# spectralcode/OCTproZ

Measured on AMD Instinct MI355X. Metric: A-scans/s, higher is better.
Workload: dtype f32

## Files before the change

octproz_amd/csrc/kernels.h:

```cpp
#pragma once
#ifndef __HIPCC_RTC__
#include <hip/hip_runtime.h>
#endif
#include <stdint.h>

#include "fft_regs.h"

namespace oct {

enum { IN_U8 = 0, IN_U16 = 1, IN_U32 = 2, IN_F32 = 3, IN_P12U = 4, IN_P12S = 5, IN_I16 = 6 };
enum { RS_NONE = 0, RS_LINEAR = 1, RS_CUBIC = 2, RS_LANCZOS = 3 };

struct FusedArgs {
	const void* raw;
	float* out;
	f2* spectrum;
	const float4* lut;
	const f2* twiddle;
	const f2* meanLine;
	unsigned numLines;
	unsigned linesInBuffer;
	unsigned ascansPerBscan;
	int bitshift;
	int rollingW;
// ... 350 lines not shown
		for (int m = 0; m < NB; m++) {
			const int b = lane + 64 * m;
			const int j0 = (b / NS) * (NS * R) + (b & (NS - 1));
			float* wb = plane + j0 + K * (j0 >> 5);
#pragma unroll
			for (int u = 0; u < R; u++) wb[u * NS + K * ((u * NS) >> 5)] = c ? v[m + u * NB].y : v[m + u * NB].x;
		}
		wave_sync_lds();
#pragma unroll
		for (int q = 0; q < P; q++) (c ? ny : nx)[q] = rb[(64 + 2 * K) * q];
		wave_sync_lds();
	}
#pragma unroll
	for (int q = 0; q < P; q++) v[q] = f2{nx[q], ny[q]};
}

template <int LOG2N> struct Plan;
template <> struct Plan<8>  { static constexpr int R0 = 4,  R1 = 4,  R2 = 4,  R3 = 4; static constexpr bool PERM = false; };
template <> struct Plan<9>  { static constexpr int R0 = 8,  R1 = 8,  R2 = 8,  R3 = 1; static constexpr bool PERM = false; };
template <> struct Plan<10> { static constexpr int R0 = 16, R1 = 16, R2 = 4,  R3 = 1; static constexpr bool PERM = true; };
template <> struct Plan<11> { static constexpr int R0 = 32, R1 = 16, R2 = 4,  R3 = 1; static constexpr bool PERM = false; };
template <> struct Plan<12> { static constexpr int R0 = 64, R1 = 16, R2 = 4,  R3 = 1; static constexpr bool PERM = false; };

template <int LOG2N> constexpr int twiddle_count() {
	typedef Plan<LOG2N> PL;
	int n = 0, ns = PL::R0;
	n += (PL::R1 - 1) * ns; ns *= PL::R1;
	n += (PL::R2 - 1) * ns; ns *= PL::R2;
	if (PL::R3 > 1) n += (PL::R3 - 1) * ns;
	return n;
}
template <int LOG2N> struct LastRadix { static constexpr int value = Plan<LOG2N>::R3 == 1 ? Plan<LOG2N>::R2 : Plan<LOG2N>::R3; };

OCT_DEV void perm_swap32(float& a, float& b) {
	const auto r = __builtin_amdgcn_permlane32_swap(__builtin_bit_cast(unsigned, a), __builtin_bit_cast(unsigned, b), false, false);
	const unsigned r0 = r[0], r1 = r[1];
	a = __builtin_bit_cast(float, r0);
	b = __builtin_bit_cast(float, r1);
}
OCT_DEV void perm_swap16(float& a, float& b) {
	const auto r = __builtin_amdgcn_permlane16_swap(__builtin_bit_cast(unsigned, a), __builtin_bit_cast(unsigned, b), false, false);
	const unsigned r0 = r[0], r1 = r[1];
	a = __builtin_bit_cast(float, r0);
	b = __builtin_bit_cast(float, r1);
}
OCT_DEV void perm_exchange16x4(f2 (&v)[16]) {
#pragma unroll
	for (int m = 0; m < 4; m++) {
		float x[4], y[4];
#pragma unroll
		for (int c = 0; c < 4; c++) { x[c] = v[4 * m + c].x; y[c] = v[4 * m + c].y; }
		perm_swap32(x[0], x[2]); perm_swap32(x[1], x[3]); perm_swap32(y[0], y[2]); perm_swap32(y[1], y[3]);
		perm_swap16(x[0], x[1]); perm_swap16(x[2], x[3]); perm_swap16(y[0], y[1]); perm_swap16(y[2], y[3]);
#pragma unroll
		for (int c = 0; c < 4; c++) v[4 * m + c] = f2{x[c], y[c]};
	}
	f2 w[16];
#pragma unroll
	for (int m = 0; m < 4; m++)
#pragma unroll
		for (int a = 0; a < 4; a++) w[m + 4 * a] = v[4 * m + a];
#pragma unroll
	for (int i = 0; i < 16; i++) v[i] = w[i];
}
template <int P> OCT_DEV void perm_exchange(f2 (&v)[P]) {
	if constexpr (P == 16) perm_exchange16x4(v);
}
OCT_DEV void perm_exchange32x2(f2 (&v)[32]) {
	f2 w[32];
#pragma unroll
	for (int m = 0; m < 2; m++)
#pragma unroll
		for (int mp = 0; mp < 8; mp++) {
			float ax = v[m + 4 * mp].x, ay = v[m + 4 * mp].y, bx = v[m + 4 * mp + 2].x, by = v[m + 4 * mp + 2].y;
			perm_swap32(ax, bx);
			perm_swap32(ay, by);
			w[mp + 8 * (2 * m)] = f2{ax, ay};
			w[mp + 8 * (2 * m + 1)] = f2{bx, by};
		}
#pragma unroll
	for (int i = 0; i < 32; i++) v[i] = w[i];
}

template <int LOG2N> OCT_DEV int fft_bin(int lane, int m, int u) {
	constexpr int N = 1 << LOG2N, RL = LastRadix<LOG2N>::value;
	return lane + 64 * m + u * (N / RL);
}
template <int LOG2N, bool PRUNE, bool REGTW = false, bool REGTW3 = false, int PRIO2 = -1>
OCT_DEV void fft_wave(f2 (&v)[(1 << LOG2N) / 64], f2* xbuf, const f2* tw, int lane, const f32x4* twr = nullptr) {
	constexpr int N = 1 << LOG2N;
	typedef Plan<LOG2N> PL;
	constexpr int R0 = PL::R0, R1 = PL::R1, R2 = PL::R2, R3 = PL::R3;
	static_assert(R0 * R1 * R2 * R3 == N, "plan");
	constexpr int T1 = 0, T2 = T1 + (R1 - 1) * R0, T3 = T2 + (R2 - 1) * R0 * R1;
	constexpr int P = N / 64;
	if constexpr (Cfg<LOG2N>::PLANAR) {
		static_assert(R1 == 16 && R2 == 4 && R3 == 1 && P == R0, "planar plans: P x 16 x 4 with the whole first pass in the lane");
		float* plane = reinterpret_cast<float*>(xbuf);
		fft_pass<N, R0, 1, false, false, false>(v, xbuf, tw, lane);
		exchange_planar<N, R0>(v, plane, lane);
		fft_pass<N, R1, R0, false, false, false>(v, xbuf, tw + T1, lane);
		if constexpr (P == 32) {
			perm_exchange32x2(v);
		} else {
			f2 w[P];
#pragma unroll
			for (int m = 0; m < 4; m++)
#pragma unroll
				for (int u = 0; u < 16; u++) w[(u + 16 * m) % P] = v[(m + 4 * u) % P];
#pragma unroll
			for (int i = 0; i < P; i++) v[i] = w[i];
		}
		fft_pass<N, R2, R0 * R1, false, false, PRUNE>(v, xbuf, tw + T2, lane);
		return;
	}
	fft_pass<N, R0, 1, false, true, false>(v, xbuf, tw, lane);
	if constexpr (PL::PERM) {
		static_assert(!PL::PERM || (R3 == 1 && R2 == 4 && R1 == 16 && P == 16), "permlane exchange: 16-point lanes, radix 16 then 4");
		fft_pass<N, R1, R0, true, false, false, 2, REGTW, false, PRIO2>(v, xbuf, tw, lane, twr);
		perm_exchange<P>(v);
		fft_pass<N, R2, R0 * R1, false, false, PRUNE, 3, REGTW, REGTW3>(v, xbuf, tw + 8 * 16 * 2, lane, twr);
	} else if constexpr (R3 == 1) {
		fft_pass<N, R1, R0, true, true, false>(v, xbuf, tw + T1, lane);
		fft_pass<N, R2, R0 * R1, true, false, PRUNE>(v, xbuf, tw + T2, lane);
	} else {
		fft_pass<N, R1, R0, true, true, false>(v, xbuf, tw + T1, lane);
		fft_pass<N, R2, R0 * R1, true, true, false>(v, xbuf, tw + T2, lane);
		fft_pass<N, R3, R0 * R1 * R2, true, false, PRUNE>(v, xbuf, tw + T3, lane);
	}
}

template <int LOG2N> constexpr int tw_lds_bytes() { return Plan<LOG2N>::PERM ? (8 * 16 + 6 * 64) * 16 : (twiddle_count<LOG2N>() * 8 + 15) & ~15; }
template <int LOG2N>
OCT_DEV void fill_twiddles(f2* tw, const f2* g, int tid, int threads) {
	if constexpr (Plan<LOG2N>::PERM) {
		typedef Plan<LOG2N> PL;
		constexpr int T2 = (PL::R1 - 1) * PL::R0;
		f32x4* p2 = reinterpret_cast<f32x4*>(tw);
		f32x4* p3 = p2 + 8 * 16;
		for (int i = tid; i < 8 * 16; i += threads) {
			const int c = i >> 4, k = i & 15;
			const f2 w0 = c ? g[(2 * c - 1) * 16 + k] : f2{1.0f, 0.0f}, w1 = g[(2 * c) * 16 + k];
			p2[i] = f32x4{w0.x, w0.y, w1.x, w1.y};
		}
		for (int i = tid; i < 6 * 64; i += threads) {
			const int c = i >> 6, l = i & 63, i0 = 2 * c, i1 = 2 * c + 1;
			const f2 w0 = g[T2 + (i0 % 3) * 256 + l + 64 * (i0 / 3)], w1 = g[T2 + (i1 % 3) * 256 + l + 64 * (i1 / 3)];
			p3[i] = f32x4{w0.x, w0.y, w1.x, w1.y};
		}
	} else {
		for (int i = tid; i < twiddle_count<LOG2N>(); i += threads) tw[i] = g[i];
	}
}
template <int LOG2N, int RS> constexpr int mean_lds_bytes() { return KCfg<LOG2N, RS>::MEAN_REGS ? 0 : (1 << LOG2N) * 4; }
template <int LOG2N, int RS, bool ROLL = false> constexpr int lut_lds_bytes() { return (!Cfg<LOG2N>::LDS_LUT || KCfg<LOG2N, RS>::REGTAB || KCfg<LOG2N, RS, ROLL>::REGLIN) ? 0 : (1 << LOG2N) * (KCfg<LOG2N, RS>::CW ? 24 : 12) + (KCfg<LOG2N, RS>::LZ_LDS ? (1 << LOG2N) * 64 : 0); }
template <int LOG2N, int RS, bool ROLL> constexpr int block_lds_bytes() {
	return tw_lds_bytes<LOG2N>() + mean_lds_bytes<LOG2N, RS>() + lut_lds_bytes<LOG2N, RS, ROLL>() + KCfg<LOG2N, RS, ROLL>::WAVES * wave_lds_bytes<(1 << LOG2N), ROLL>();
}

OCT_DEV unsigned flipped_row(const FusedArgs& a, unsigned line) {
	const unsigned b = line / a.ascansPerBscan, as = line - b * a.ascansPerBscan;
	return ((b & 1u) == 0u && (b + 2u) * a.ascansPerBscan <= a.linesInBuffer) ? b * a.ascansPerBscan + (a.ascansPerBscan - 1u - as) : line;
}
template <bool> OCT_DEV void ef_flush(const FusedArgs& a, float acc, unsigned first, unsigned stride, int lane, unsigned count) {
	if ((unsigned)lane < count) {
		const unsigned line = first + (unsigned)lane * stride;
		a.dispEnFace[a.dispEnFaceLast - (a.flip ? flipped_row(a, line) : line)] = acc;
	}
}

enum { MODE_ROLL = 1, MODE_SPECTRUM = 2, MODE_LOG = 4, MODE_BG = 8, MODE_DISP = 16, MODE_SINUS = 32 };
template <int MODE, int LOG2N, int RS> constexpr int sinus_lds_bytes() {
	constexpr bool ROLL = (MODE & MODE_ROLL) != 0;
	constexpr int want = KCfg<LOG2N, RS, ROLL>::WAVES * (1 << LOG2N) * 2;
	return (MODE & MODE_SINUS) != 0 && block_lds_bytes<LOG2N, RS, ROLL>() + bg_lds_bytes<MODE, (1 << LOG2N)>() + want <= 160 * 1024 ? want : 0;
}
template <int MODE, int LOG2N, int RS> constexpr bool sinus_prev_lds() { return sinus_lds_bytes<MODE, LOG2N, RS>() > 0; }
OCT_DEV float sinus_blend(float f0, float f1, float frac) {
#pragma clang fp contract(off)
	const float d = f1 - f0;
	const float t = d * frac;
	return f0 + t;
}

struct SinusWalk {
	typedef const __attribute__((address_space(4))) u32x4 ent_t;
	ent_t* ent;
	unsigned M, total, blk, A, lines, units;
	int flip;
	unsigned sBlk, sT, sTEnd, sI2, sBA, sBA0, sBB, next;
	bool sFl;
	u32x4 e0, e1, e2;
	OCT_DEV bool flipped(unsigned bb) const { return flip && (bb & 1u) == 0u && (bb + 2u) * A <= lines; }
	OCT_DEV unsigned row(unsigned ba, bool fl, uint32_t x) const { const unsigned pp = x & 0xffffu; return ba + (fl ? A - 1u - pp : pp); }
	OCT_DEV unsigned wrap(unsigned i) const { return i + 1u == M ? 0u : i + 1u; }
	OCT_DEV bool valid() const { return sBlk * blk + 1u < total; }
	OCT_DEV unsigned enter() {
		const unsigned g0 = sBlk * blk, last = total - 1u;
		sTEnd = min(blk, last - g0);
		sT = 0;
		const unsigned bb = g0 / M, i0 = g0 - bb * M, i1 = wrap(i0);
		e0 = ent[i0];
		e1 = ent[i1];
		sI2 = wrap(i1);
		sBA0 = bb * A;
		sBB = i1 == 0u ? bb + 1u : bb;
		sBA = sBB * A;
		sFl = flipped(sBB);
		return row(sBA0, flipped(bb), e0.x);
	}
	OCT_DEV unsigned begin(const FusedArgs& a, unsigned first, unsigned unitsInGrid) {
		ent = reinterpret_cast<ent_t*>(reinterpret_cast<uintptr_t>(a.sinEnt));
		M = a.sinM; total = a.sinTotal; blk = a.sinBlk; A = a.ascansPerBscan; lines = a.linesInBuffer; flip = a.flip; units = unitsInGrid;
		sBlk = first; sT = sTEnd = sI2 = sBA = sBA0 = sBB = 0; next = 0xFFFFFFFFu; sFl = false;
		e0 = e1 = e2 = u32x4{0u, 0u, 0u, 0u};
		return valid() ? enter() : 0xFFFFFFFFu;
	}
	OCT_DEV void load_ahead() { e2 = ent[sI2]; }
	OCT_DEV unsigned peek_next() { next = sT < sTEnd ? row(sBA, sFl, e1.x) : 0xFFFFFFFFu; return next; }
	OCT_DEV unsigned advance(bool* newBlock) {
		*newBlock = false;
		if (sT < sTEnd) {
			sT++;
			e0 = e1; sBA0 = sBA;
			e1 = e2;
			if (sI2 == 0u) { sBB++; sBA += A; sFl = flipped(sBB); }
			sI2 = wrap(sI2);
			return next;
		}
		sBlk += units;
		if (!valid()) return 0xFFFFFFFFu;
		*newBlock = true;
		return enter();
	}
	OCT_DEV unsigned out_row() const { return sBA0 + (e0.x >> 16); }
	OCT_DEV void pair(float* f0, float* f1, bool* st0, bool* st1, bool* raw) const {
		const uint32_t b0 = e0.y, b1 = e0.z;
		*f0 = __builtin_bit_cast(float, b0);
		*f1 = __builtin_bit_cast(float, b1);
		const unsigned r0 = out_row();
		const bool p = sT > 0u && *f0 >= 0.0f;
		*st0 = p && r0 + 1u != lines;
		*st1 = p && *f1 >= 0.0f && r0 + 2u != lines;
		*raw = sBA0 + (e0.x & 0xffffu) + 1u == lines;
	}
};

template <int LOG2N, int INTYPE, int RS, int MODE>
__global__ __launch_bounds__((KCfg<LOG2N, RS, (MODE & 1) != 0>::WAVES) * 64, (KCfg<LOG2N, RS, (MODE & 1) != 0>::MINW)) void oct_fused_kernel(const FusedArgs a) {
	constexpr int N = 1 << LOG2N, P = N / 64;
	constexpr int WAVES = KCfg<LOG2N, RS, (MODE & MODE_ROLL) != 0>::WAVES, THREADS = WAVES * 64;
	constexpr bool LDS_LUT = Cfg<LOG2N>::LDS_LUT, CW = KCfg<LOG2N, RS>::CW, MEAN_REGS = KCfg<LOG2N, RS>::MEAN_REGS, REGTAB = KCfg<LOG2N, RS>::REGTAB;
	constexpr bool REGLIN = KCfg<LOG2N, RS, (MODE & 1) != 0>::REGLIN && RS != RS_LANCZOS;
	constexpr int RL = LastRadix<LOG2N>::value, NBL = P / RL;
	constexpr bool ROLL = (MODE & MODE_ROLL) != 0, SPECTRUM = (MODE & MODE_SPECTRUM) != 0, LOGSCALE = (MODE & MODE_LOG) != 0;
	constexpr bool SINUS = (MODE & MODE_SINUS) != 0;
	static_assert(!(SINUS && (SPECTRUM || (MODE & MODE_DISP) != 0 || RS == RS_LANCZOS)), "sinusoidal correction in the store: image output of the raw-row variants, display frames by the extraction kernel");
	typedef Chunk<INTYPE, N> CH;
	constexpr int SPL = CH::SPL, CB = CH::BYTES, NL = N / (64 * SPL);
	static_assert(!(RS == RS_LANCZOS && INTYPE != IN_F32 && INTYPE != IN_U16), "Lanczos: prepared float buffer or raw uint16 rows");
	static_assert(!(RS == RS_LANCZOS && (MODE & MODE_ROLL) != 0), "Lanczos taps cross line borders: the rolling average of the neighbour rows comes prepared");
	static_assert(!(ROLL && INTYPE != IN_U16), "in-kernel rolling average: uint16 rows only (everything else comes prepared)");
	static_assert(N / (64 * SPL) >= 1, "a row holds at least one chunk per lane");
	extern __shared__ __attribute__((aligned(16))) char smem[];
	f2* tw = reinterpret_cast<f2*>(smem);
	f2* meanL = reinterpret_cast<f2*>(smem + tw_lds_bytes<LOG2N>());
	float* rhoL = reinterpret_cast<float*>(smem + tw_lds_bytes<LOG2N>() + mean_lds_bytes<LOG2N, RS>());
	f32x4* cwL = reinterpret_cast<f32x4*>(rhoL);
	f2* wphL = reinterpret_cast<f2*>(smem + tw_lds_bytes<LOG2N>() + mean_lds_bytes<LOG2N, RS>() + N * (CW ? 16 : 4));
	constexpr bool LZ_LDS = KCfg<LOG2N, RS>::LZ_LDS;
	f32x4* lzL = reinterpret_cast<f32x4*>(smem + tw_lds_bytes<LOG2N>() + mean_lds_bytes<LOG2N, RS>() + N * 12);
	const int tid = threadIdx.x, lane = tid & 63;
	const int wave = __builtin_amdgcn_readfirstlane(tid >> 6);
	char* wbase = smem + tw_lds_bytes<LOG2N>() + mean_lds_bytes<LOG2N, RS>() + lut_lds_bytes<LOG2N, RS, ROLL>() + wave * wave_lds_bytes<N, ROLL>();
	float* row = reinterpret_cast<float*>(wbase);
	f2* xbuf = reinterpret_cast<f2*>(wbase);

	const float* termL = reinterpret_cast<const float*>(smem + block_lds_bytes<LOG2N, RS, ROLL>());
	constexpr bool SINUS_PREV_LDS = sinus_prev_lds<MODE, LOG2N, RS>();
	float* sPrevL = reinterpret_cast<float*>(smem + block_lds_bytes<LOG2N, RS, ROLL>() + bg_lds_bytes<MODE, N>()) + wave * (N / 2);
	float sPrevR[SINUS && !SINUS_PREV_LDS ? P / 2 : 1];
	if constexpr (SINUS && !SINUS_PREV_LDS) {
#pragma unroll
		for (int i = 0; i < P / 2; i++) sPrevR[i] = 0.0f;
	}
	if constexpr ((MODE & MODE_BG) != 0) fill_bg_term(reinterpret_cast<float*>(smem + block_lds_bytes<LOG2N, RS, ROLL>()), a.bgTerm, N / 2, tid, THREADS);
	fill_twiddles<LOG2N>(tw, a.twiddle, tid, THREADS);
	if constexpr (LZ_LDS) {
		const f32x4* g = reinterpret_cast<const f32x4*>(a.lanczosW);
		for (int u = tid; u < N * 4; u += THREADS) lzL[u] = g[((u & 63) + 64 * (u >> 8)) * 4 + ((u >> 6) & 3)];
	}
	if constexpr (!MEAN_REGS)
		for (int i = tid; i < N / 2; i += THREADS) meanL[i] = a.subtractMean ? a.meanLine[i] : f2{0.0f, 0.0f};
	if constexpr (LDS_LUT && !REGTAB && !REGLIN) {
		for (int i = tid; i < N; i += THREADS) {
			const float4 t = a.lut[i];
			wphL[CW ? (((i >> 7) << 6) + (i & 63)) * 2 + ((i >> 6) & 1) : i] = f2{t.y * t.z, t.y * t.w};
			if constexpr (CW) {
				const float4 w = a.cubicW[i];
				cwL[i] = f32x4{w.x, w.y, w.z, w.w};
			} else {
				rhoL[i] = t.x;
			}
		}
	}
	__syncthreads();

	const unsigned wavesTotal = gridDim.x * (unsigned)WAVES;
#ifndef OCT_DISP_BLOCK
#define OCT_DISP_BLOCK 16
#endif
	constexpr unsigned BLK = (MODE & MODE_DISP) != 0 ? (unsigned)OCT_DISP_BLOCK : 1u;
	static_assert(BLK >= 1 && BLK <= 64, "a block's en-face values live in the lanes of one register");
	const unsigned blockStride = wavesTotal * BLK;
	const unsigned blk = blockIdx.x;
	unsigned line = (blk * (unsigned)WAVES + (unsigned)wave) * BLK;
	unsigned inBlock = 0;
	SinusWalk sw;
	if constexpr (SINUS) line = sw.begin(a, blk * (unsigned)WAVES + (unsigned)wave, wavesTotal);
	auto next_line = [&](unsigned ln, unsigned pos) -> unsigned {
		if (BLK > 1u && pos + 1u < BLK) return ln + 1u;
		return ln - pos + blockStride;
	};
	const unsigned lineEnd = a.numLines;
	const __amdgpu_buffer_rsrc_t lutR = make_rsrc(a.lut, N * 16u);
	const __amdgpu_buffer_rsrc_t lanczosR = make_rsrc(a.lanczosW, N * 64u);
	const unsigned rowBytes = (unsigned)(N / SPL) * CB;
	const uint32_t shift = a.bitshift ? 4u : 0u;
	u32x4 pre[NL];
	if constexpr (RS != RS_LANCZOS) {
		if (line < lineEnd) {
			const __amdgpu_buffer_rsrc_t rawR = make_rsrc(reinterpret_cast<const char*>(a.raw) + (size_t)line * rowBytes, rowBytes);
#pragma unroll
			for (int i = 0; i < NL; i++) pre[i] = load_chunk<INTYPE, N>(rawR, lane * CB, i * 64 * CB);
		}
	}
	auto advance = [&]() {
		if constexpr (SINUS) {
			bool newBlock;
			line = sw.advance(&newBlock);
			if (newBlock && line < lineEnd) {
				const __amdgpu_buffer_rsrc_t rawR = make_rsrc(reinterpret_cast<const char*>(a.raw) + (size_t)line * rowBytes, rowBytes);
#pragma unroll
				for (int i = 0; i < NL; i++) pre[i] = load_chunk<INTYPE, N>(rawR, lane * CB, i * 64 * CB);
			}
		} else {
			line = next_line(line, inBlock);
			inBlock = (inBlock + 1u == BLK) ? 0u : inBlock + 1u;
		}
	};
	f2 mreg[MEAN_REGS && !SPECTRUM ? P / 2 : 1];
	if constexpr (MEAN_REGS && !SPECTRUM) {
#pragma unroll
		for (int u = 0; u < RL / 2; u++)
#pragma unroll
			for (int m = 0; m < NBL; m++)
				mreg[m + u * NBL] = a.subtractMean ? a.meanLine[fft_bin<LOG2N>(lane, m, u)] : f2{0.0f, 0.0f};
	}
	float* rowl = row + ROW_OFF + lane;
	uint32_t tapA[CW ? P : 1];
	typedef __attribute__((address_space(3))) const float lds_cfloat;
	const uint32_t tapBase = __builtin_amdgcn_readfirstlane(
	    (uint32_t)(uintptr_t)(__attribute__((address_space(3))) float*)(row + ROW_OFF - 1));

	if constexpr (CW) {
#pragma unroll
		for (int q = 0; q < P; q++) tapA[q] = tapBase + 4u * (uint32_t)(int)a.lut[lane + 64 * q].x;
	}
	f32x4 cwR[REGTAB ? P : 1];
	f2 wphR[REGTAB || REGLIN ? P : 1];
	float fracR[REGLIN && RS == RS_LINEAR ? P : 1];
	uint32_t tapL[REGLIN && RS == RS_LINEAR ? P : 1];
	if constexpr (REGLIN) {
#pragma unroll
		for (int q = 0; q < P; q++) {
			const float4 t = a.lut[lane + 64 * q];
			wphR[q] = f2{t.y * t.z, t.y * t.w};
			if constexpr (RS == RS_LINEAR) {
				fracR[q] = __builtin_amdgcn_fractf(t.x);
				tapL[q] = tapBase + 4u * (uint32_t)(int)t.x + 4u;
			}
		}
	}
	constexpr bool TW3 = (REGTAB || REGLIN) && LOG2N == 10 && !ROLL && INTYPE != IN_F32;
	constexpr bool TW2 = (REGTAB || REGLIN) && LOG2N == 10 && !ROLL;
	f32x4 tw2R[TW2 ? (TW3 ? 14 : 8) : 1];
	if constexpr (REGTAB) {
#pragma unroll
		for (int q = 0; q < P; q++) {
			const float4 t = a.lut[lane + 64 * q];
			wphR[q] = f2{t.y * t.z, t.y * t.w};
			const float4 w = a.cubicW[lane + 64 * q];
			cwR[q] = f32x4{w.x, w.y, w.z, w.w};
		}
	}
	if constexpr (TW2) {
#pragma unroll
		for (int c = 0; c < 8; c++) tw2R[c] = reinterpret_cast<const f32x4*>(tw)[c * 16 + (lane & 15)];
	}
	if constexpr (TW3) {
#pragma unroll
		for (int c = 0; c < 6; c++) tw2R[8 + c] = reinterpret_cast<const f32x4*>(tw)[8 * 16 + c * 64 + lane];
	}
	float rollCnt[ROLL ? 8 : 1], rollRc[ROLL ? 8 : 1];
	if constexpr (ROLL) {
#pragma unroll
		for (int e = 0; e < 8; e++) {
			const int j = 4 * lane + (e < 4 ? 0 : 256 * (NL - 1)) + (e & 3);
			const int lo = max(0, j - a.rollingW + 1), hi = min(N - 1, j + a.rollingW);
			rollCnt[e] = (float)(hi - lo + 1);
			rollRc[e] = __fdiv_rn(1.0f, rollCnt[e]);
		}
	}
	constexpr bool DISP = (MODE & MODE_DISP) != 0;
	static_assert(!(DISP && SPECTRUM), "display frames are copies of the image");
	const unsigned efIdx = DISP ? __builtin_amdgcn_readfirstlane(a.dispEnFaceBin >> 6) : 0u, efLane = DISP ? __builtin_amdgcn_readfirstlane(a.dispEnFaceBin & 63u) : 0u;
	float efAcc = 0.0f;
	unsigned efCount = 0, efFirst = line;
	prologue_wait();
	while (line < lineEnd) {
		if constexpr (SINUS) sw.load_ahead();
		if constexpr (RS != RS_LANCZOS) {
			bool staged = false;
			if constexpr (ROLL) {
				const int W = a.rollingW;
				{
					staged = true;
					uint32_t* pfx = reinterpret_cast<uint32_t*>(row + N + 2 * ROW_OFF);
					uint32_t base = 0;
#pragma unroll
					for (int i = 0; i < NL; i++) {
						const uint4 x = chunk_to_uint(pre[i], 0, shift);
						const uint32_t tot = x.x + x.y + x.z + x.w;
						const uint32_t incl = wave_inclusive_scan(tot);
						const uint32_t p3 = base + incl, p2 = p3 - x.w, p1 = p2 - x.z, p0 = p1 - x.y;
						*reinterpret_cast<uint4*>(&pfx[ROLL_PAD + 4 * lane + 256 * i]) = uint4{p0, p1, p2, p3};
						base += (uint32_t)__builtin_amdgcn_readlane((int)incl, 63);
					}
					static_assert(ROLL_PAD == 256, "pad writes: four entries per lane");
					*reinterpret_cast<uint4*>(&pfx[4 * lane]) = uint4{0u, 0u, 0u, 0u};
					*reinterpret_cast<uint4*>(&pfx[ROLL_PAD + N + 4 * lane]) = uint4{base, base, base, base};
					wave_sync_lds();
					const uint32_t* hiP = pfx + ROLL_PAD + 4 * lane + W;
					const uint32_t* loP = pfx + ROLL_PAD + 4 * lane - W;
					const float cntIn = (float)(2 * W), rcIn = __fdiv_rn(1.0f, cntIn);
					const bool quad = (W & 3) == 0;
					const bool fast = a.rollExact == 2;
					uint32_t wsAll[NL][4];
					if (quad) {
						uint4 h4[NL], l4[NL];
#pragma unroll
						for (int i = 0; i < NL; i++) { h4[i] = *reinterpret_cast<const uint4*>(hiP + 256 * i); l4[i] = *reinterpret_cast<const uint4*>(loP + 256 * i); }
#pragma unroll
						for (int i = 0; i < NL; i++) { wsAll[i][0] = h4[i].x - l4[i].x; wsAll[i][1] = h4[i].y - l4[i].y; wsAll[i][2] = h4[i].z - l4[i].z; wsAll[i][3] = h4[i].w - l4[i].w; }
					} else {
#pragma unroll
						for (int i = 0; i < NL; i++)
#pragma unroll
							for (int c = 0; c < 4; c++) wsAll[i][c] = hiP[256 * i + c] - loP[256 * i + c];
					}
					__builtin_amdgcn_sched_barrier(0);
#pragma unroll
					for (int i = 0; i < NL; i++) {
						float o[4];
						const uint4 x = chunk_to_uint(pre[i], 0, shift);
						const uint32_t xs[4] = {x.x, x.y, x.z, x.w};
						uint32_t ws[4] = {wsAll[i][0], wsAll[i][1], wsAll[i][2], wsAll[i][3]};
						const bool whole = fast && i > 0 && i < NL - 1;
						if (whole) {
#pragma unroll
							for (int c = 0; c < 4; c++)
								o[c] = __builtin_fmaf((float)ws[c], -rcIn, (float)xs[c]);
						} else
#pragma unroll
						for (int c = 0; c < 4; c++) {
							const float sum = (float)ws[c];
							float cnt = cntIn, rc = rcIn;
							if (i == NL - 1) { cnt = rollCnt[4 + c]; rc = rollRc[4 + c]; }
							else if (i == 0) { cnt = rollCnt[c]; rc = rollRc[c]; }
							const float q0 = sum * rc;
							const float q = __builtin_fmaf(__builtin_fmaf(-q0, cnt, sum), rc, q0);
							o[c] = (float)xs[c] - q;
						}
						*reinterpret_cast<float4*>(&row[ROW_OFF + 4 * lane + 256 * i]) = float4{o[0], o[1], o[2], o[3]};
						if constexpr (RS == RS_CUBIC) { if (i == 0 && lane == 0) row[ROW_OFF - 1] = o[1]; }
					}
				}
			}
			if (!staged) {
#pragma unroll
				for (int i = 0; i < NL; i++) {
#pragma unroll
					for (int h = 0; h < SPL / 4; h++) {
						const float4 f = chunk_to_float<INTYPE>(pre[i], h, shift);
						*reinterpret_cast<float4*>(&row[ROW_OFF + SPL * lane + 64 * SPL * i + 4 * h]) = f;
						if constexpr (RS == RS_CUBIC) { if (i == 0 && h == 0 && lane == 0) row[ROW_OFF - 1] = f.y; }
					}
				}
			}
			unsigned next;
			if constexpr (SINUS) next = sw.peek_next();
			else next = next_line(line, inBlock);
			if (next < lineEnd) {
				const __amdgpu_buffer_rsrc_t rawR = make_rsrc(reinterpret_cast<const char*>(a.raw) + (size_t)next * rowBytes, rowBytes);
#pragma unroll
				for (int i = 0; i < NL; i++) pre[i] = load_chunk<INTYPE, N>(rawR, lane * CB, i * 64 * CB);
			}
		} else {
			const long long S = (long long)a.linesInBuffer * N;
			long long off = (long long)line * N;
			if (off < 8) off = 8;
			if (off > S - 9) off = S - 9;
			if constexpr (INTYPE == IN_U16) {
				const uint16_t* g = reinterpret_cast<const uint16_t*>(a.raw) + (off - 8);
				const long long left = (S - (off - 8)) * 2;
				const __amdgpu_buffer_rsrc_t haloR = make_rsrc(g, (uint32_t)(left < (long long)(N + 16) * 2 ? left : (long long)(N + 16) * 2));
				constexpr int UNITS = (N + 16) / 8;
#pragma unroll
				for (int i = 0; i < (UNITS + 63) / 64; i++) {
					const int u = lane + 64 * i;
					if (u < UNITS) {
						const u32x4 c = __builtin_bit_cast(u32x4, buf_load128(haloR, u * 16, 0));
						*reinterpret_cast<float4*>(&row[ROW_OFF - 8 + 8 * u]) = chunk_to_float<IN_U16>(c, 0, shift);
						*reinterpret_cast<float4*>(&row[ROW_OFF - 8 + 8 * u + 4]) = chunk_to_float<IN_U16>(c, 1, shift);
					}
				}
			} else {
			const float* g = reinterpret_cast<const float*>(a.raw) + (off - 8);
			const long long left = (S - (off - 8)) * 4;
			const __amdgpu_buffer_rsrc_t haloR = make_rsrc(g, (uint32_t)(left < (long long)(N + 16) * 4 ? left : (long long)(N + 16) * 4));
			constexpr int UNITS = (N + 16) / 4;
#pragma unroll
			for (int i = 0; i < (UNITS + 63) / 64; i++) {
				const int u = lane + 64 * i;
				if (u < UNITS) {
					const f32x4 f = buf_load128(haloR, u * 16, 0);
					*reinterpret_cast<float4*>(&row[ROW_OFF - 8 + 4 * u]) = float4{f.x, f.y, f.z, f.w};
				}
			}
			}
		}
		wave_sync_lds();

		if constexpr (Cfg<LOG2N>::PRIO) __builtin_amdgcn_s_setprio(OCT_PRIO_GATHER);
		f2 v[P];
		f32x4 wph2;
		constexpr bool LZ_GLOBAL = RS == RS_LANCZOS && !LZ_LDS;
		constexpr int LZ_AHEAD = (LOG2N == 11 && OCT_LANCZOS_AHEAD > 1) ? 1 : OCT_LANCZOS_AHEAD;
		f32x4 lzw[LZ_GLOBAL ? LZ_AHEAD + 1 : 1][4];
		if constexpr (LZ_GLOBAL) {
#pragma unroll
			for (int q = 0; q < LZ_AHEAD && q < P; q++)
#pragma unroll
				for (int c = 0; c < 4; c++) lzw[q][c] = buf_load128(lanczosR, lane * 64, q * 4096 + c * 16);
		}
// ... 232 lines not shown
```

octproz_amd/csrc/pipe_calib.hip:

```cpp
#include "pipe_internal.h"

using namespace octimpl;

namespace oct {

__global__ __launch_bounds__(256) void oct_tap_weights_kernel(const float4* lut, float4* cw, int n) {
	const int i = blockIdx.x * blockDim.x + threadIdx.x;
	if (i >= n) return;
	const double p = (double)__builtin_amdgcn_fractf(lut[i].x);
	const double w0 = 0.5 * p * ((2.0 - p) * p - 1.0), w2 = 0.5 * p * ((4.0 - 3.0 * p) * p + 1.0), w3 = 0.5 * p * p * (p - 1.0);
	cw[i] = float4{(float)w0, (float)(1.0 - w0 - w2 - w3), (float)w2, (float)w3};
}

}

namespace octimpl {

float4 lutEntry(const octpipe* h, int j, bool unitPhasor) {
	const int N = h->N;
	const OctPipeParams& p = h->params;
	float rho = p.resampling ? h->resample[j] : (float)j;
	if (!(rho >= 0.0f)) rho = 0.0f;
	if (rho > (float)(N - 3)) rho = (float)(N - 3);
	const bool disp = p.dispersionCompensation && !unitPhasor;
	float4 e;
	e.x = rho;
	e.y = p.windowing ? h->window[j] : 1.0f;
	e.z = disp ? h->phase[2 * j] : 1.0f;
	e.w = disp ? h->phase[2 * j + 1] : 0.0f;
	return e;
}

void lanczosWeights(const std::vector<float4>& lut, std::vector<float>& w) {
	const int N = (int)lut.size();
	w.resize((size_t)N * 16);
	const float PI_F = 3.141592654f, PI_OVER_8 = 0.3926990817f;
	for (int j = 0; j < N; ++j) {
		const float rho = lut[j].x;
		const int n0 = (int)rho;
		for (int i = -7; i <= 8; ++i) {
			const float x = rho - (float)(n0 + i), ax = fabsf(x);
			const float s1 = sinf(PI_F * ax) / (PI_F * ax), s8 = sinf(PI_OVER_8 * ax) / (PI_OVER_8 * ax);
			w[(size_t)j * 16 + (size_t)(i + 7)] = (ax < 0.00001f) ? 1.0f : (s1 * s8);
		}
	}
}

int uploadLut(octpipe* h) {
	const int N = h->N;
	std::vector<float4> lut(N), plain(h->mixed ? N : 0);
	const OctPipeParams& p = h->params;
	for (int j = 0; j < N; ++j) {
		float4 e = lutEntry(h, j, false);
		if (h->mixed) plain[j] = e;
		if (h->bluestein) {
			const double ang = 3.14159265358979323846 * (double)(((long long)j * j) % (2LL * N)) / (double)N;
			const double cr = cos(ang), ci = sin(ang), pr = e.z, pi = e.w;
			e.z = (float)(pr * cr - pi * ci);
			e.w = (float)(pr * ci + pi * cr);
		}
		lut[j] = e;
	}
	HIP_TRY(hipMemcpyAsync(h->d_lut, lut.data(), sizeof(float4) * N, hipMemcpyHostToDevice, h->stream));
	if (!h->d_cubicW) HIP_TRY(hipMalloc((void**)&h->d_cubicW, sizeof(float4) * N));
	hipLaunchKernelGGL(oct::oct_tap_weights_kernel, dim3((N + 255) / 256), dim3(256), 0, h->stream, h->d_lut, h->d_cubicW, N);
	HIP_TRY(hipGetLastError());
	if (h->mixed) HIP_TRY(hipMemcpyAsync(h->d_lutPlain, plain.data(), sizeof(float4) * N, hipMemcpyHostToDevice, h->stream));
	if (p.resampling && p.resamplingInterpolation == OCTPIPE_INTERP_LANCZOS) {
		std::vector<float> w;
		lanczosWeights(lut, w);
		if (h->mixed) {
			std::vector<float> r(w.size());
			for (int j = 0; j < N; ++j)
				for (int c = 0; c < 4; ++c) std::memcpy(&r[(size_t)oct::mixed1664_lanczos_unit(j, c) * 4], &w[(size_t)j * 16 + (size_t)c * 4], 16);
			w.swap(r);
		}
		if (!h->d_lanczosW) HIP_TRY(hipMalloc((void**)&h->d_lanczosW, sizeof(float) * w.size()));
		HIP_TRY(hipMemcpyAsync(h->d_lanczosW, w.data(), sizeof(float) * w.size(), hipMemcpyHostToDevice, h->stream));
		HIP_TRY(hipStreamSynchronize(h->stream));
	}
	HIP_TRY(hipStreamSynchronize(h->stream));
	h->lutDirty = false;
	return OCTPIPE_OK;
}

int fusedTwiddles(int log2n, std::vector<f2>& tw) {
	int radices[4];
	const int count = oct::fused_twiddle_plan(log2n, radices);
	if (count < 0) return fail(OCTPIPE_ERR_UNSUPPORTED, "no FFT plan for this samplesPerLine");
	tw.assign((size_t)count, f2{0.0f, 0.0f});
	size_t pos = 0;
	int ns = radices[0];
	for (int pass = 1; pass < 4; ++pass) {
		const int R = radices[pass];
		if (R <= 1) break;
		for (int t = 1; t < R; ++t)
			for (int k = 0; k < ns; ++k) {
				const double ang = 2.0 * 3.14159265358979323846 * (double)t * (double)k / ((double)ns * R);
				tw[pos++] = f2{(float)cos(ang), (float)sin(ang)};
			}
		ns *= R;
	}
	return OCTPIPE_OK;
}

int uploadTwiddles(octpipe* h) {
	std::vector<f2> tw;
	const int rc = fusedTwiddles(h->log2n, tw);
	if (rc) return rc;
	HIP_TRY(hipMalloc(&h->d_twiddle, sizeof(f2) * tw.size()));
	return uploadSync(h, h->d_twiddle, tw.data(), sizeof(f2) * tw.size());
}

int uploadBluesteinTables(octpipe* h) {
	const int N = h->N, M = 1 << h->log2n;
	const double pi = 3.14159265358979323846;
	std::vector<double> cr(N), ci(N), wr(M), wi(M);
	for (int m = 0; m < N; ++m) {
		const double ang = pi * (double)(((long long)m * m) % (2LL * N)) / (double)N;
		cr[m] = cos(ang); ci[m] = sin(ang);
	}
	for (int j = 0; j < M; ++j) { wr[j] = cos(2.0 * pi * j / M); wi[j] = sin(2.0 * pi * j / M); }
	std::vector<f2> filter(M), chirp(N);
	for (int k = 0; k < M; ++k) {
		double sr = cr[0], si = -ci[0];
		for (int m = 1; m < N; ++m) {
			const double t = 2.0 * wr[(int)(((long long)m * k) % M)];
			sr += cr[m] * t;
			si -= ci[m] * t;
		}
		filter[k] = f2{(float)sr, (float)si};
	}
	for (int k = 0; k < N; ++k) chirp[k] = f2{(float)(cr[k] / M), (float)(ci[k] / M)};
	HIP_TRY(hipMalloc((void**)&h->d_filter, sizeof(f2) * M));
	HIP_TRY(hipMalloc((void**)&h->d_outChirp, sizeof(f2) * N));
	int rc = uploadSync(h, h->d_filter, filter.data(), sizeof(f2) * M);
	return rc ? rc : uploadSync(h, h->d_outChirp, chirp.data(), sizeof(f2) * N);
}

int bindFftLibrary(octpipe* h) {
	const char* names[] = {"libhipfft.so.0", "libhipfft.so"};
	for (const char* n : names) if (!h->fftLib) h->fftLib = dlopen(n, RTLD_NOW | RTLD_NOLOAD);
	for (const char* n : names) if (!h->fftLib) h->fftLib = dlopen(n, RTLD_NOW | RTLD_LOCAL);
	if (!h->fftLib) return fail(OCTPIPE_ERR_UNSUPPORTED, "samplesPerLine outside 256..4096 / 8..2047 needs libhipfft.so, which could not be loaded");
	h->fftPlan1d = reinterpret_cast<decltype(h->fftPlan1d)>(dlsym(h->fftLib, "hipfftPlan1d"));
	h->fftSetStream = reinterpret_cast<decltype(h->fftSetStream)>(dlsym(h->fftLib, "hipfftSetStream"));
	h->fftExecC2C = reinterpret_cast<decltype(h->fftExecC2C)>(dlsym(h->fftLib, "hipfftExecC2C"));
	h->fftDestroy = reinterpret_cast<decltype(h->fftDestroy)>(dlsym(h->fftLib, "hipfftDestroy"));
	if (!h->fftPlan1d || !h->fftSetStream || !h->fftExecC2C || !h->fftDestroy) return fail(OCTPIPE_ERR_UNSUPPORTED, "libhipfft.so lacks the C2C entry points");
	return OCTPIPE_OK;
}

int uploadTeamTables(octpipe* h) {
	std::vector<f2> tw((size_t)oct::team_twiddle_count(h->log2n));
	size_t pos = 0;
	const int radix[3] = {16, oct::team_last_radix(h->log2n), 2}, ns[3] = {16, 256, 4096};
	const int passes = h->log2n == 13 ? 3 : 2;
	for (int pass = 0; pass < passes; ++pass)
		for (int t = 1; t < radix[pass]; ++t)
			for (int k = 0; k < ns[pass]; ++k) {
				const double ang = 2.0 * 3.14159265358979323846 * (double)t * (double)k / ((double)ns[pass] * radix[pass]);
				tw[pos++] = f2{(float)cos(ang), (float)sin(ang)};
			}
	if (pos != tw.size()) return fail(OCTPIPE_ERR_DEVICE, "team twiddle table size mismatch");
	HIP_TRY(hipMalloc((void**)&h->d_twTeam, sizeof(f2) * tw.size()));
	return uploadSync(h, h->d_twTeam, tw.data(), sizeof(f2) * tw.size());
}

int uploadMixedNTable(octpipe* h) {
	const int N = h->N;
	std::vector<f2> tw((size_t)N);
	for (int j = 0; j < N; ++j) {
		const double ang = 2.0 * 3.14159265358979323846 * (double)j / (double)N;
		tw[(size_t)j] = f2{(float)cos(ang), (float)sin(ang)};
	}
	HIP_TRY(hipMalloc((void**)&h->d_twMixedN, sizeof(f2) * tw.size()));
	return uploadSync(h, h->d_twMixedN, tw.data(), sizeof(f2) * tw.size());
}

int uploadMixedTables(octpipe* h) {
	const int N = 1664, N1 = 32, N2 = 52;
	std::vector<f2> tw((size_t)N1 * N2);
	for (int k1 = 0; k1 < N1; ++k1)
		for (int n2 = 0; n2 < N2; ++n2) {
			const double ang = 2.0 * 3.14159265358979323846 * (double)((k1 * n2) % N) / (double)N;
			tw[(size_t)k1 * N2 + n2] = f2{(float)cos(ang), (float)sin(ang)};
		}
	HIP_TRY(hipMalloc((void**)&h->d_twMixed, sizeof(f2) * tw.size()));
	if (int rcUp = uploadSync(h, h->d_twMixed, tw.data(), sizeof(f2) * tw.size())) return rcUp;
	HIP_TRY(hipMalloc((void**)&h->d_lutPlain, sizeof(float4) * N));
	std::vector<f2> tt((size_t)oct::team1664_twiddle_count());
	size_t pos = 0;
	const int radix[2] = {16, 8}, ns[2] = {13, 208};
	for (int pass = 0; pass < 2; ++pass)
		for (int t = 1; t < radix[pass]; ++t)
			for (int k = 0; k < ns[pass]; ++k) {
				const double ang = 2.0 * 3.14159265358979323846 * (double)t * (double)k / ((double)ns[pass] * radix[pass]);
				tt[pos++] = f2{(float)cos(ang), (float)sin(ang)};
			}
	if (pos != tt.size()) return fail(OCTPIPE_ERR_DEVICE, "team twiddle table size mismatch");
	HIP_TRY(hipMalloc((void**)&h->d_twTeam, sizeof(f2) * tt.size()));
	return uploadSync(h, h->d_twTeam, tt.data(), sizeof(f2) * tt.size());
}

}

extern "C" {

int octpipe_update_resample_curve(octpipe_t* h, const float* curve, int size) {
	if (!h) return fail(OCTPIPE_ERR_INVALID_ARGUMENT, "null handle");
	if (curve && size > 0 && size <= h->N) {
		std::memcpy(h->resample.data(), curve, sizeof(float) * (size_t)size);
		h->lutDirty = true;
	}
	return OCTPIPE_OK;
}

int octpipe_update_dispersion_curve(octpipe_t* h, const float* curve, int size) {
	if (!h) return fail(OCTPIPE_ERR_INVALID_ARGUMENT, "null handle");
	if (curve && size > 0 && size <= h->N) {
		std::memcpy(h->dispersion.data(), curve, sizeof(float) * (size_t)size);
		octhost::dispersive_phase(h->dispersion.data(), (unsigned)h->N, h->phase.data());
		h->lutDirty = true;
	}
	return OCTPIPE_OK;
}

int octpipe_update_window_curve(octpipe_t* h, const float* curve, int size) {
	if (!h) return fail(OCTPIPE_ERR_INVALID_ARGUMENT, "null handle");
	if (curve && size > 0 && size <= h->N) {
		std::memcpy(h->window.data(), curve, sizeof(float) * (size_t)size);
		h->lutDirty = true;
	}
	return OCTPIPE_OK;
}

int octpipe_update_postprocess_background(octpipe_t* h, const float* background, int size) {
	if (!h) return fail(OCTPIPE_ERR_INVALID_ARGUMENT, "null handle");
	if (background && size > 0 && size <= h->N / 2) {
		int rc = setDevice(h); if (rc) return rc;
		std::memcpy(h->h_postBg.data(), background, sizeof(float) * (size_t)size);
		HIP_TRY(hipMemcpyAsync(h->d_postBg, h->h_postBg.data(), sizeof(float) * (size_t)size, hipMemcpyHostToDevice, h->stream));
		h->bgVersion++;
		HIP_TRY(hipStreamSynchronize(h->stream));
	}
	return OCTPIPE_OK;
}

int octpipe_copy_postprocess_background_to_host(octpipe_t* h, float* background, int size) {
	if (!h || !background || size <= 0 || size > h->N / 2) return fail(OCTPIPE_ERR_INVALID_ARGUMENT, "invalid argument");
	int rc = setDevice(h); if (rc) return rc;
	HIP_TRY(hipMemcpyAsync(background, h->d_postBg, sizeof(float) * (size_t)size, hipMemcpyDeviceToHost, h->stream));
	HIP_TRY(hipStreamSynchronize(h->stream));
	return OCTPIPE_OK;
}
// ... 68 lines not shown
```

Baseline: 857.0 million.

## Batch kernel prologue table loads into registers and prepack twiddles on host

```diff
diff --git a/octproz_amd/csrc/kernels.h b/octproz_amd/csrc/kernels.h
--- a/octproz_amd/csrc/kernels.h
+++ b/octproz_amd/csrc/kernels.h
@@ -526,6 +526,28 @@
 		for (int i = tid; i < twiddle_count<LOG2N>(); i += threads) tw[i] = g[i];
 	}
 }
+template <int LOG2N> constexpr int packed_twiddle_units() { return Plan<LOG2N>::PERM ? 8 * 16 + 6 * 64 : 0; }
+template <int UNITS, int THREADS> struct TableFetch {
+	static constexpr int IT = (UNITS + THREADS - 1) / THREADS;
+	static constexpr bool RAGGED = UNITS % THREADS != 0;
+	f32x4 r[IT];
+	template <typename S> OCT_DEV void load(const void* g, int tid, S&& src) {
+		const f32x4* p = reinterpret_cast<const f32x4*>(g);
+#pragma unroll
+		for (int k = 0; k < IT; k++) {
+			const int i = tid + k * THREADS;
+			r[k] = p[src(RAGGED && k == IT - 1 ? min(i, UNITS - 1) : i)];
+		}
+	}
+	OCT_DEV void load(const void* g, int tid) { load(g, tid, [](int i) { return i; }); }
+	template <typename F> OCT_DEV void each(int tid, F&& f) const {
+#pragma unroll
+		for (int k = 0; k < IT; k++) {
+			const int i = tid + k * THREADS;
+			if (!RAGGED || k < IT - 1 || i < UNITS) f(i, r[k]);
+		}
+	}
+};
 template <int LOG2N, int RS> constexpr int mean_lds_bytes() { return KCfg<LOG2N, RS>::MEAN_REGS ? 0 : (1 << LOG2N) * 4; }
 template <int LOG2N, int RS, bool ROLL = false> constexpr int lut_lds_bytes() { return (!Cfg<LOG2N>::LDS_LUT || KCfg<LOG2N, RS>::REGTAB || KCfg<LOG2N, RS, ROLL>::REGLIN) ? 0 : (1 << LOG2N) * (KCfg<LOG2N, RS>::CW ? 24 : 12) + (KCfg<LOG2N, RS>::LZ_LDS ? (1 << LOG2N) * 64 : 0); }
 template <int LOG2N, int RS, bool ROLL> constexpr int block_lds_bytes() {
@@ -658,28 +680,6 @@
 #pragma unroll
 		for (int i = 0; i < P / 2; i++) sPrevR[i] = 0.0f;
 	}
-	if constexpr ((MODE & MODE_BG) != 0) fill_bg_term(reinterpret_cast<float*>(smem + block_lds_bytes<LOG2N, RS, ROLL>()), a.bgTerm, N / 2, tid, THREADS);
-	fill_twiddles<LOG2N>(tw, a.twiddle, tid, THREADS);
-	if constexpr (LZ_LDS) {
-		const f32x4* g = reinterpret_cast<const f32x4*>(a.lanczosW);
-		for (int u = tid; u < N * 4; u += THREADS) lzL[u] = g[((u & 63) + 64 * (u >> 8)) * 4 + ((u >> 6) & 3)];
-	}
-	if constexpr (!MEAN_REGS)
-		for (int i = tid; i < N / 2; i += THREADS) meanL[i] = a.subtractMean ? a.meanLine[i] : f2{0.0f, 0.0f};
-	if constexpr (LDS_LUT && !REGTAB && !REGLIN) {
-		for (int i = tid; i < N; i += THREADS) {
-			const float4 t = a.lut[i];
-			wphL[CW ? (((i >> 7) << 6) + (i & 63)) * 2 + ((i >> 6) & 1) : i] = f2{t.y * t.z, t.y * t.w};
-			if constexpr (CW) {
-				const float4 w = a.cubicW[i];
-				cwL[i] = f32x4{w.x, w.y, w.z, w.w};
-			} else {
-				rhoL[i] = t.x;
-			}
-		}
-	}
-	__syncthreads();
-
 	const unsigned wavesTotal = gridDim.x * (unsigned)WAVES;
 #ifndef OCT_DISP_BLOCK
 #define OCT_DISP_BLOCK 16
@@ -723,13 +723,72 @@
 			inBlock = (inBlock + 1u == BLK) ? 0u : inBlock + 1u;
 		}
 	};
+	constexpr bool TW3 = (REGTAB || REGLIN) && LOG2N == 10 && !ROLL && INTYPE != IN_F32;
+	constexpr bool TW2 = (REGTAB || REGLIN) && LOG2N == 10 && !ROLL;
+	constexpr bool TW_LDS = !(TW2 && TW3);
+	constexpr bool PERM = Plan<LOG2N>::PERM;
+	static_assert(twiddle_count<LOG2N>() % 2 == 0, "the canonical tables are whole 16-byte units");
+	const f32x4* twPacked = reinterpret_cast<const f32x4*>(a.twiddle + twiddle_count<LOG2N>());
+	f32x4 tw2R[TW2 ? (TW3 ? 14 : 8) : 1];
+	if constexpr (TW2) {
+		const __amdgpu_buffer_rsrc_t twR = make_rsrc(twPacked, packed_twiddle_units<LOG2N>() * 16u);
+#pragma unroll
+		for (int c = 0; c < 8; c++) tw2R[c] = buf_load128(twR, (lane & 15) * 16, c * 256);
+		if constexpr (TW3) {
+#pragma unroll
+			for (int c = 0; c < 6; c++) tw2R[8 + c] = buf_load128(twR, lane * 16, 8 * 256 + c * 1024);
+		}
+	}
+	TableFetch<TW_LDS ? (PERM ? packed_twiddle_units<LOG2N>() : twiddle_count<LOG2N>() / 2) : 1, THREADS> twF;
+	if constexpr (TW_LDS) twF.load(PERM ? reinterpret_cast<const void*>(twPacked) : reinterpret_cast<const void*>(a.twiddle), tid);
 	f2 mreg[MEAN_REGS && !SPECTRUM ? P / 2 : 1];
 	if constexpr (MEAN_REGS && !SPECTRUM) {
 #pragma unroll
 		for (int u = 0; u < RL / 2; u++)
 #pragma unroll
-			for (int m = 0; m < NBL; m++)
-				mreg[m + u * NBL] = a.subtractMean ? a.meanLine[fft_bin<LOG2N>(lane, m, u)] : f2{0.0f, 0.0f};
+			for (int m = 0; m < NBL; m++) mreg[m + u * NBL] = a.meanLine[fft_bin<LOG2N>(lane, m, u)];
+	}
+	TableFetch<!MEAN_REGS ? N / 4 : 1, THREADS> meanF;
+	if constexpr (!MEAN_REGS) meanF.load(a.meanLine, tid);
+	f32x4 lutT[REGTAB || REGLIN ? P : 1], cwT[REGTAB ? P : 1];
+	float rhoT[CW && !REGTAB ? P : 1];
+	if constexpr (REGTAB || REGLIN) {
+#pragma unroll
+		for (int q = 0; q < P; q++) lutT[q] = buf_load128(lutR, lane * 16, q * 1024);
+	} else if constexpr (CW) {
+#pragma unroll
+		for (int q = 0; q < P; q++) rhoT[q] = a.lut[lane + 64 * q].x;
+	}
+	if constexpr (REGTAB) {
+		const __amdgpu_buffer_rsrc_t cubicR = make_rsrc(a.cubicW, N * 16u);
+#pragma unroll
+		for (int q = 0; q < P; q++) cwT[q] = buf_load128(cubicR, lane * 16, q * 1024);
+	}
+	constexpr bool BG = (MODE & MODE_BG) != 0, LUT_LDS = LDS_LUT && !REGTAB && !REGLIN;
+	TableFetch<BG ? N / 8 : 1, THREADS> bgF;
+	if constexpr (BG) bgF.load(a.bgTerm, tid);
+	TableFetch<LZ_LDS ? N * 4 : 1, THREADS> lzF;
+	if constexpr (LZ_LDS) lzF.load(a.lanczosW, tid, [](int u) { return ((u & 63) + 64 * (u >> 8)) * 4 + ((u >> 6) & 3); });
+	TableFetch<LUT_LDS ? N : 1, THREADS> lutF, cwF;
+	if constexpr (LUT_LDS) lutF.load(a.lut, tid);
+	if constexpr (LUT_LDS && CW) cwF.load(a.cubicW, tid);
+	__builtin_amdgcn_sched_barrier(0);
+
+	if constexpr (BG) bgF.each(tid, [&](int i, f32x4 u) { reinterpret_cast<f32x4*>(smem + block_lds_bytes<LOG2N, RS, ROLL>())[i] = u; });
+	if constexpr (TW_LDS) twF.each(tid, [&](int i, f32x4 u) { reinterpret_cast<f32x4*>(tw)[i] = u; });
+	if constexpr (LZ_LDS) lzF.each(tid, [&](int i, f32x4 u) { lzL[i] = u; });
+	if constexpr (!MEAN_REGS) meanF.each(tid, [&](int i, f32x4 u) { reinterpret_cast<f32x4*>(meanL)[i] = a.subtractMean ? u : f32x4{0.0f, 0.0f, 0.0f, 0.0f}; });
+	if constexpr (LUT_LDS) {
+		lutF.each(tid, [&](int i, f32x4 t) {
+			wphL[CW ? (((i >> 7) << 6) + (i & 63)) * 2 + ((i >> 6) & 1) : i] = f2{t.y * t.z, t.y * t.w};
+			if constexpr (!CW) rhoL[i] = t.x;
+		});
+		if constexpr (CW) cwF.each(tid, [&](int i, f32x4 w) { cwL[i] = w; });
+	}
+	if constexpr (BG || TW_LDS || LZ_LDS || !MEAN_REGS || LUT_LDS) __syncthreads();
+	if constexpr (MEAN_REGS && !SPECTRUM) {
+#pragma unroll
+		for (int i = 0; i < P / 2; i++) mreg[i] = a.subtractMean ? mreg[i] : f2{0.0f, 0.0f};
 	}
 	float* rowl = row + ROW_OFF + lane;
 	uint32_t tapA[CW ? P : 1];
@@ -737,9 +796,12 @@
 	const uint32_t tapBase = __builtin_amdgcn_readfirstlane(
 	    (uint32_t)(uintptr_t)(__attribute__((address_space(3))) float*)(row + ROW_OFF - 1));
 
-	if constexpr (CW) {
-#pragma unroll
-		for (int q = 0; q < P; q++) tapA[q] = tapBase + 4u * (uint32_t)(int)a.lut[lane + 64 * q].x;
+	if constexpr (REGTAB) {
+#pragma unroll
+		for (int q = 0; q < P; q++) tapA[q] = tapBase + 4u * (uint32_t)(int)lutT[q].x;
+	} else if constexpr (CW) {
+#pragma unroll
+		for (int q = 0; q < P; q++) tapA[q] = tapBase + 4u * (uint32_t)(int)rhoT[q];
 	}
 	f32x4 cwR[REGTAB ? P : 1];
 	f2 wphR[REGTAB || REGLIN ? P : 1];
@@ -748,7 +810,7 @@
 	if constexpr (REGLIN) {
 #pragma unroll
 		for (int q = 0; q < P; q++) {
-			const float4 t = a.lut[lane + 64 * q];
+			const f32x4 t = lutT[q];
 			wphR[q] = f2{t.y * t.z, t.y * t.w};
 			if constexpr (RS == RS_LINEAR) {
 				fracR[q] = __builtin_amdgcn_fractf(t.x);
@@ -756,25 +818,13 @@
 			}
 		}
 	}
-	constexpr bool TW3 = (REGTAB || REGLIN) && LOG2N == 10 && !ROLL && INTYPE != IN_F32;
-	constexpr bool TW2 = (REGTAB || REGLIN) && LOG2N == 10 && !ROLL;
-	f32x4 tw2R[TW2 ? (TW3 ? 14 : 8) : 1];
 	if constexpr (REGTAB) {
 #pragma unroll
 		for (int q = 0; q < P; q++) {
-			const float4 t = a.lut[lane + 64 * q];
+			const f32x4 t = lutT[q];
 			wphR[q] = f2{t.y * t.z, t.y * t.w};
-			const float4 w = a.cubicW[lane + 64 * q];
-			cwR[q] = f32x4{w.x, w.y, w.z, w.w};
-		}
-	}
-	if constexpr (TW2) {
-#pragma unroll
-		for (int c = 0; c < 8; c++) tw2R[c] = reinterpret_cast<const f32x4*>(tw)[c * 16 + (lane & 15)];
-	}
-	if constexpr (TW3) {
-#pragma unroll
-		for (int c = 0; c < 6; c++) tw2R[8 + c] = reinterpret_cast<const f32x4*>(tw)[8 * 16 + c * 64 + lane];
+			cwR[q] = cwT[q];
+		}
 	}
 	float rollCnt[ROLL ? 8 : 1], rollRc[ROLL ? 8 : 1];
 	if constexpr (ROLL) {
diff --git a/octproz_amd/csrc/pipe_calib.hip b/octproz_amd/csrc/pipe_calib.hip
--- a/octproz_amd/csrc/pipe_calib.hip
+++ b/octproz_amd/csrc/pipe_calib.hip
@@ -101,6 +101,19 @@
 			}
 		ns *= R;
 	}
+	if (log2n == 10 && radices[0] == 16 && radices[1] == 16 && radices[2] == 4) {
+		const size_t T2 = 15 * 16;
+		tw.reserve((size_t)count + 2 * (8 * 16 + 6 * 64));
+		for (int i = 0; i < 8 * 16; ++i) {
+			const int c = i >> 4, k = i & 15;
+			tw.push_back(c ? tw[(size_t)(2 * c - 1) * 16 + k] : f2{1.0f, 0.0f});
+			tw.push_back(tw[(size_t)(2 * c) * 16 + k]);
+		}
+		for (int i = 0; i < 6 * 64; ++i) {
+			const int c = i >> 6, l = i & 63;
+			for (int e = 2 * c; e <= 2 * c + 1; ++e) tw.push_back(tw[T2 + (size_t)(e % 3) * 256 + l + 64 * (e / 3)]);
+		}
+	}
 	return OCTPIPE_OK;
 }
 
```

New measurement: 854.4 million. No clear change (-0.3%).
